# megvii-research/basedet

Hardware: AMD Instinct MI355X
Metric: images/sec training RetinaNet-R50-FPN 1333x800 (higher is better)
Workload: dtype bf16; 1 GPU; retinanet_r50_800x1344 train step (fwd+bwd+allreduce+SGD), DummyLoader boxes, random-init weights, inputs resident in HBM; per_gpu_batch=16, global_batch=16, parallelism=dp1

## Files before the change

### basedet_amd/_lib.py

```python
import ctypes as C
import os

import torch

_HERE = os.path.dirname(os.path.abspath(__file__))
LIB_PATH = os.environ.get("BASEDET_HIP_LIB") or os.path.join(_HERE, "lib", "libbasedet_hip.so")

BD_MAX_SEGS = 8
ABI_VERSION = 118
EPI_RELU, EPI_ADD_BEFORE, EPI_ADD_AFTER, EPI_MASK, EPI_SPARSE = 1, 2, 4, 8, 16


class BasedetHipError(RuntimeError):
    pass


class ConvDesc(C.Structure):
    _fields_ = [
        ("N", C.c_int32), ("Cin", C.c_int32), ("Cout", C.c_int32), ("R", C.c_int32), ("S", C.c_int32),
        ("stride", C.c_int32), ("pad", C.c_int32), ("nseg", C.c_int32),
        ("Hi", C.c_int32 * BD_MAX_SEGS), ("Wi", C.c_int32 * BD_MAX_SEGS),
        ("Ho", C.c_int32 * BD_MAX_SEGS), ("Wo", C.c_int32 * BD_MAX_SEGS),
        ("in_off", C.c_int32 * BD_MAX_SEGS), ("out_off", C.c_int32 * BD_MAX_SEGS),
        ("in_pix_per_img", C.c_int32), ("out_pix_per_img", C.c_int32),
        ("route", C.c_int32 * 4), ("sr_seed", C.c_uint32),
        ("gskip", C.c_int32), ("gskip_ws", C.c_void_p), ("gskip_ws_bytes", C.c_size_t),
        ("gskip_gmap", C.c_void_p), ("gskip_gmap_bytes", C.c_size_t), ("gskip_dxmap", C.c_void_p), ("gskip_dxmap_bytes", C.c_size_t),
        ("gskip_dx_clean", C.c_int32),
        ("fwd_map", C.c_void_p), ("fwd_map_bytes", C.c_size_t), ("fwd_clean", C.c_int32),
    ]


class PackDesc(C.Structure):
    _fields_ = [("w", C.c_void_p), ("row_scale", C.c_void_p), ("w_fwd", C.c_void_p), ("w_dgrad", C.c_void_p),
                ("Cout", C.c_int32), ("RS", C.c_int32), ("Cin", C.c_int32), ("block_start", C.c_int32)]


class ImageDesc(C.Structure):
    _fields_ = [("offset", C.c_int64), ("src_h", C.c_int32), ("src_w", C.c_int32), ("dst_h", C.c_int32), ("dst_w", C.c_int32),
                ("flip", C.c_int32), ("reserved_", C.c_int32 * 1)]


AFFINE_BRIGHTNESS, AFFINE_CONTRAST, AFFINE_SATURATION, AFFINE_LIGHTING = 1, 2, 4, 8

# ... 7 lines not shown
_P, _I, _L, _F, _Z = C.c_void_p, C.c_int, C.c_int64, C.c_float, C.c_size_t
_D = C.POINTER(ConvDesc)

SIGNATURES = {
    "bd_last_error_string": (C.c_char_p, []),
    "bd_version": (_I, []),
    "bd_conv_last_kernel": (C.c_char_p, []),
    "bd_probe_mfma_rate": (_I, [C.c_double, C.POINTER(C.c_double), C.POINTER(C.c_double), _P]),
    "bd_probe_kernel_clock": (_I, [C.c_char_p, _I, C.POINTER(C.c_double), C.POINTER(C.c_double)]),
    "bd_conv2d_fwd": (_I, [_D, _P, _P, _P, _P, _P, _I, _P]),
    "bd_conv2d_dgrad": (_I, [_D, _P, _P, _P, _P, _P, _I, _P]),
    "bd_conv2d_dgrad_gskip_bytes": (_Z, [_D]),
    "bd_conv2d_gskip_map_bytes": (_Z, [_D, _I]),
    "bd_gskip_map_scan": (_I, [_D, _I, _P, _P, _Z, _P]),
    "bd_fwd_live_map_bytes": (_Z, [_D]),
    "bd_fwd_live_maps": (_I, [_D, _P, _I, _I, C.POINTER(C.c_void_p), _Z, _I, _P]),
    "bd_conv2d_fwd_bits": (_I, [_D, _P, _P, _P, _P, _P, _P, _I, _P]),
    "bd_conv2d_fwd_ex": (_I, [_D, _P, _P, _P, _P, _P, _P, _P, _F, _I, _P]),
    "bd_conv2d_dgrad_ex": (_I, [_D, _P, _P, _P, _P, _P, _P, _P, _F, _I, _P]),
    "bd_conv2d_dgrad_bits": (_I, [_D, _P, _P, _P, _P, _P, _I, _P]),
    "bd_conv2d_wgrad_workspace_bytes": (_Z, [_D]),
    "bd_conv2d_wgrad": (_I, [_D, _P, _P, _P, _P, _I, _P, _Z, _P]),
    "bd_conv2d_wgrad_bias_workspace_bytes": (_Z, [_D]),
    "bd_conv2d_wgrad_bias": (_I, [_D, _P, _P, _P, _P, _P, _I, _P, _Z, _P]),
    "bd_fpn_deconv_pack": (_I, [_P, _I, _P, _P, _P]),
    "bd_fpn_deconv_fwd": (_I, [_P, _P, _P, _P, _I, _I, _I, _I, _I, _I, _P]),
    "bd_fpn_deconv_dgrad": (_I, [_P, _P, _P, _P, _I, _I, _I, _I, _I, _I, _P]),
    "bd_fpn_deconv_wgrad_workspace_bytes": (_Z, [_I, _I, _I, _I]),
    "bd_fpn_deconv_wgrad": (_I, [_P, _P, _P, _I, _P, _Z, _I, _I, _I, _I, _I, _I, _P]),
    "bd_deform_conv_fwd": (_I, [_P, _P, _P, _P, _P] + [_I] * 12 + [_P]),
    "bd_deform_conv_wgrad_workspace_bytes": (_Z, [_I] * 5),
# ... 222 lines not shown
```

### basedet_amd/csrc/conv3x3_pp128.hip

```cpp
#include "conv3x3_pp128_body.h"

namespace {
using namespace pp128;

struct PSeg { int patch_start, H, W, pw, src_off, dst_off; };

struct PParams {
    const bf16_raw* src;
    const bf16_raw* w;
    const float* bias;
    const bf16_raw* add;
    const bf16_raw* mask;
    bf16_raw* dst;
    int CK, CO, flags, nseg;
    int src_ppi, dst_ppi;
    unsigned src_bytes;
    int patches_per_img, total_patches, n_tiles;
    int patch_begin;
    PSeg seg[MAX_SEG];
};


template <int MODE, int TCO>
__global__ __launch_bounds__(512, 1) void conv3x3_pp128_kernel(const PParams p) {
    extern __shared__ __attribute__((aligned(16))) unsigned char smem[];
    pp128::body<MODE, TCO>(p, smem, (int)blockIdx.x, (int)gridDim.x, p.patch_begin, p.total_patches, p.n_tiles);
}

}

extern BD_KNOB int g_patch_pp128;
int bd_conv3x3_pp128_launch_range(const bd_conv_desc* d, int mode, const void* src, const void* w, const float* bias, const void* add,
                                  const void* mask, void* dst, int flags, hipStream_t stream, int patch_begin, int patch_end, int tco) {
    PParams p{};
    p.CK = mode == 0 ? d->Cin : d->Cout;
    p.CO = mode == 0 ? d->Cout : d->Cin;
    p.src_ppi = mode == 0 ? d->in_pix_per_img : d->out_pix_per_img;
    p.dst_ppi = mode == 0 ? d->out_pix_per_img : d->in_pix_per_img;
    if (p.CK % 8 != 0 || p.CO % 8 != 0) return 1;
    if ((long long)d->N * p.src_ppi * p.CK * 2 >= 0x7fffffffll || (long long)d->N * p.dst_ppi >= 0x7fffffffll ||
        (long long)p.CO * 9 * p.CK >= 0x7fffffffll) return 1;
    p.src = (const bf16_raw*)src; p.w = (const bf16_raw*)w; p.bias = bias;
    p.add = (const bf16_raw*)add; p.mask = (const bf16_raw*)mask; p.dst = (bf16_raw*)dst;
    p.flags = flags; p.nseg = d->nseg;
    p.src_bytes = (unsigned)((long long)d->N * p.src_ppi * p.CK * 2);
    int ps = 0;
    for (int s = 0; s < d->nseg; ++s) {
        PSeg& sg = p.seg[s];
        sg.patch_start = ps; sg.H = d->Ho[s]; sg.W = d->Wo[s]; sg.pw = cdiv(d->Wo[s], PW);
        sg.src_off = mode == 0 ? d->in_off[s] : d->out_off[s];
        sg.dst_off = mode == 0 ? d->out_off[s] : d->in_off[s];
        ps += cdiv(d->Ho[s], PH) * sg.pw;
    }
    p.patches_per_img = ps;
    p.total_patches = patch_end >= 0 ? patch_end : ps * d->N;
    p.patch_begin = patch_begin;
    const bool small = tco ? tco == 64 : p.CO <= 64;
    if (!tco && (g_patch_pp128 < 0 || (g_patch_pp128 == 0 && !small))) return 1;
    p.n_tiles = cdiv(p.CO, small ? 64 : 128);
    const int grid = cdiv(p.total_patches - p.patch_begin, NPATCH) * p.n_tiles;
    if (grid <= 0) return 0;
    BD_ONCE_PER_DEVICE(
        (void)hipFuncSetAttribute(reinterpret_cast<const void*>(&conv3x3_pp128_kernel<0, 128>), hipFuncAttributeMaxDynamicSharedMemorySize, Tile<128>::LDS_BYTES);
        (void)hipFuncSetAttribute(reinterpret_cast<const void*>(&conv3x3_pp128_kernel<1, 128>), hipFuncAttributeMaxDynamicSharedMemorySize, Tile<128>::LDS_BYTES);
        (void)hipFuncSetAttribute(reinterpret_cast<const void*>(&conv3x3_pp128_kernel<0, 64>), hipFuncAttributeMaxDynamicSharedMemorySize, Tile<64>::LDS_BYTES);
        (void)hipFuncSetAttribute(reinterpret_cast<const void*>(&conv3x3_pp128_kernel<1, 64>), hipFuncAttributeMaxDynamicSharedMemorySize, Tile<64>::LDS_BYTES));
    if (!tco) bd_note_kernel("conv3x3_pp128_kernel");
    if (small) {
        if (mode == 0) hipLaunchKernelGGL((conv3x3_pp128_kernel<0, 64>), dim3(grid), dim3(512), Tile<64>::LDS_BYTES, stream, p);
        else hipLaunchKernelGGL((conv3x3_pp128_kernel<1, 64>), dim3(grid), dim3(512), Tile<64>::LDS_BYTES, stream, p);
    } else {
        if (mode == 0) hipLaunchKernelGGL((conv3x3_pp128_kernel<0, 128>), dim3(grid), dim3(512), Tile<128>::LDS_BYTES, stream, p);
        else hipLaunchKernelGGL((conv3x3_pp128_kernel<1, 128>), dim3(grid), dim3(512), Tile<128>::LDS_BYTES, stream, p);
    }
    return 0;
}

int bd_conv3x3_pp128_launch(const bd_conv_desc* d, int mode, const void* src, const void* w, const float* bias, const void* add,
                            const void* mask, void* dst, int flags, hipStream_t stream) {
    return bd_conv3x3_pp128_launch_range(d, mode, src, w, bias, add, mask, dst, flags, stream, 0, -1, 0);
}
```

### basedet_amd/csrc/conv3x3_pp128_body.h

```cpp
#pragma once
#include "common.h"

namespace pp128 {


constexpr int PH = 4, PW = 16, IH = PH + 2, IW = PW + 2;
constexpr int NPATCH = 4;
constexpr int XROWS = NPATCH * IH * IW;
constexpr int X_PITCH = 144;
constexpr int X_BYTES = XROWS * X_PITCH;
constexpr int XPASSES = 7;
constexpr int NSLOT = 4;
template <int TCO> struct Tile {
    static constexpr int W_SLOT = TCO * 128;
    static constexpr int W_BYTES = NSLOT * W_SLOT;
    static constexpr int LDS_BYTES = W_BYTES + X_BYTES + TCO * 4;
    static constexpr int MREP = TCO / 32;
    static constexpr int NPIECE = TCO / 64;
};
constexpr int MAX_SEG = BD_MAX_SEGS;

typedef __attribute__((address_space(3))) void lds_void_t;
typedef __attribute__((address_space(1))) const void glb_void_t;

__device__ __forceinline__ int swz(int row, int chunk) { return row * 128 + ((chunk ^ (row & 7)) << 4); }
__device__ __forceinline__ int colperm(int f) { return f < 4 ? 2 * f : (f < 12 ? 2 * (f - 4) + 1 : 2 * (f - 8)); }
__device__ __forceinline__ int xpos(int chunk) { return (chunk >> 2) * 64 + ((((chunk & 1) << 1) | ((chunk >> 1) & 1)) << 4); }

#define PP_FENCE() __builtin_amdgcn_sched_barrier(0)
#define PP_BARRIER() do { asm volatile("" ::: "memory"); __builtin_amdgcn_s_barrier(); asm volatile("" ::: "memory"); } while (0)


template <int MODE, int TCO, class P>
__device__ __forceinline__ void body(const P& p, unsigned char* smem, int bid, const int nwg, const int patch_begin, const int patch_end, const int n_tiles) {
    constexpr int TILE_CO = TCO, W_SLOT = Tile<TCO>::W_SLOT, W_BYTES = Tile<TCO>::W_BYTES, MREP = Tile<TCO>::MREP, NPIECE = Tile<TCO>::NPIECE;
    constexpr int HALF = TCO / 2;
    unsigned char* wbuf = smem;
    unsigned char* xbuf = smem + W_BYTES;
    float* sbias = reinterpret_cast<float*>(smem + W_BYTES + X_BYTES);

    const int tid = threadIdx.x, lane = tid & 63, wave = __builtin_amdgcn_readfirstlane(tid >> 6);
    const int wm = wave >> 2, wp = wave & 3;
    {
        const int q = nwg >> 3, r = nwg & 7, xcd = bid & 7;
        bid = (xcd < r ? xcd * (q + 1) : r * (q + 1) + (xcd - r) * q) + (bid >> 3);
    }
    const int pt = bid / n_tiles;
    const int ct = bid - pt * n_tiles;
    const int co0 = ct * TILE_CO;

    int py0[NPATCH], px0[NPATCH], pH[NPATCH], pWd[NPATCH];
    int psrc[NPATCH], pdst[NPATCH];
#pragma unroll
    for (int k = 0; k < NPATCH; ++k) {
        const int pid = patch_begin + pt * NPATCH + k;
        pH[k] = 0; pWd[k] = 0; py0[k] = 0; px0[k] = 0; psrc[k] = 0; pdst[k] = 0;
        if (pid < patch_end) {
            const int n = pid / p.patches_per_img;
            const int rem = pid - n * p.patches_per_img;
            int s = 0;
#pragma unroll
            for (int q = 1; q < MAX_SEG; ++q)
                if (q < p.nseg && rem >= p.seg[q].patch_start) s = q;
            const auto sg = p.seg[s];
            const int local = rem - sg.patch_start;
            const int by = local / sg.pw, bx = local - by * sg.pw;
            py0[k] = by * PH; px0[k] = bx * PW; pH[k] = sg.H; pWd[k] = sg.W;
            psrc[k] = n * p.src_ppi + sg.src_off;
            pdst[k] = n * p.dst_ppi + sg.dst_off;
        }
// ... 226 lines not shown
```

### basedet_amd/csrc/conv_igemm.hip

```cpp
#include "igemm_params.h"

using namespace igemm;

namespace {

template <int BK>
struct Cfg {
    static constexpr int CHUNKS = BK / 8;
    static constexpr int ROWS_PER_PASS = 256 / CHUNKS;
    static constexpr int PASSES = 128 / ROWS_PER_PASS;
    static constexpr int LDS_STRIDE = BK == 64 ? 160 : 64;
    static constexpr int TILE_BYTES = 128 * LDS_STRIDE;
    __device__ static __forceinline__ int off(int row, int chunk) {
        if constexpr (BK == 64) return row * LDS_STRIDE + chunk * 16;
        else return row * 64 + ((chunk ^ ((row >> 1) & 3)) << 4);
    }
};

template <int BK, bool PRE, bool BUF>
__global__ __launch_bounds__(256) void conv_igemm_kernel(const IgemmParams p) {
    using C = Cfg<BK>;
    extern __shared__ __attribute__((aligned(16))) unsigned char smem[];
    unsigned char* tiles = smem;
    unsigned int* s_tapmask = reinterpret_cast<unsigned int*>(smem);
// ... 373 lines not shown
}
BD_KNOB int g_use_patch3x3 = 1;
#ifdef BD_AB_SKIP
BD_KNOB int g_skip_s2_3x3 = 0;
#endif
BD_KNOB int g_bk32_for_1x1 = 1;
BD_KNOB int g_bk32_s2 = 1;

}


int bd_conv3x3_patch_launch(const bd_conv_desc* d, int mode, const void* src, const void* w, const float* bias,
                            const void* add, const void* mask, void* dst, int flags, hipStream_t stream);
bool bd_conv3x3_pp_maps_ok(const bd_conv_desc* d, int flags, const void* add, const void* dst);
bool bd_conv3x3_pp_fwd_map_ok(const bd_conv_desc* d, int flags, const void* add);

extern BD_KNOB int g_patch_dma;
extern BD_KNOB int g_patch_pp;
extern BD_KNOB int g_patch_pp128;
extern BD_KNOB int g_conv1x1_s2;
extern BD_KNOB int g_pp_tail_split;
extern BD_KNOB int g_pp_persistent;
static int bd_route_patch3x3(int enable) {
#ifdef BD_AB_SKIP
    g_skip_s2_3x3 = (enable >> 4) & 1;
#else
    if ((enable >> 4) & 1) {
        bd_set_error("bd_conv_desc.route[1]: bit 4 (skip the 3x3 / stride-2 launches: a timing A/B that leaves stale outputs) exists in "
                     "-DBD_AB_SKIP diagnostic builds only");
        return BD_EINVAL;
// ... 42 lines not shown
                         const unsigned* maskbits, void* dst, int flags, hipStream_t stream);
namespace {
bool is_dense_1x1(const bd_conv_desc* d) {
    return d->R == 1 && d->S == 1 && d->stride == 1 && d->pad == 0 && d->nseg == 1 && d->in_off[0] == 0 && d->out_off[0] == 0 &&
           d->in_pix_per_img == d->Hi[0] * d->Wi[0] && d->out_pix_per_img == d->Ho[0] * d->Wo[0];
}
}

static int conv2d_fwd_impl(const bd_conv_desc* d, const void* x, const void* w_packed, const float* bias, const void* add, void* y,
                           unsigned* ybits, void* y8, float q_scale, int flags, bd_stream_t stream) {
    if (int e = check_desc(d)) return e;
    BD_REQUIRE(x && w_packed && y, "conv2d_fwd: null pointer");
    BD_REQUIRE(d->Cin % 8 == 0, "conv2d_fwd: Cin=%d must be a multiple of 8", d->Cin);
    BD_REQUIRE(d->Cout % 8 == 0, "conv2d_fwd: Cout=%d must be a multiple of 8", d->Cout);
    BD_REQUIRE(!(flags & BD_EPI_MASK), "conv2d_fwd: BD_EPI_MASK is a dgrad-only flag");
    if (d->fwd_map || d->fwd_clean) {
        BD_REQUIRE(d->fwd_map && is_3x3s1(d) && g_use_patch3x3 && !ybits && !y8 && bd_conv3x3_pp_fwd_map_ok(d, flags, add),
                   "conv2d_fwd: fwd_map needs a 3x3 / stride 1 / pad 1 descriptor into more than 128 channels without residual operand on the "
                   "default route (fwd_clean needs fwd_map)");
        BD_REQUIRE(d->fwd_map_bytes >= bd_fwd_live_map_bytes(d), "conv2d_fwd: fwd_map %zu < required %zu bytes", (size_t)d->fwd_map_bytes,
                   bd_fwd_live_map_bytes(d));
    }
    if (is_dense_1x1(d) &&
        bd_conv1x1_dense_launch(x, w_packed, bias, add, nullptr, nullptr, y, ybits, y8, q_scale, 0, (long long)d->N * d->out_pix_per_img,
                                d->Cin, d->Cout, flags, (hipStream_t)stream) == 0) {
        BD_CHECK_LAUNCH("bd_conv2d_fwd(dense 1x1)");
        return BD_OK;
    }
    if (!ybits && !y8 && d->stride == 2 && d->R == 1 &&
        bd_conv1x1_s2_launch(d, 0, x, w_packed, bias, add, nullptr, nullptr, y, flags, (hipStream_t)stream) == 0) {
        BD_CHECK_LAUNCH("bd_conv2d_fwd(1x1 stride 2)");
// ... 175 lines not shown
```

### basedet_amd/csrc/gskip.hip

```cpp
#include "common.h"

namespace {

enum { GS_ANY = 1, GS_TOP = 2, GS_BOT = 4, GS_LEFT = 8, GS_RIGHT = 16, GS_TL = 32, GS_TR = 64, GS_BL = 128, GS_BR = 256 };

struct GsSeg { int patch_start, H, W, pw, off; };

struct GsParams {
    const bf16_raw* g;
    int* mask;
    int C, ppi, ph, pw_px, nseg, patches_per_img, total;
    GsSeg seg[BD_MAX_SEGS];
};

__device__ __forceinline__ int gs_level(const GsParams& p, int rem) {
    int s = 0;
#pragma unroll
    for (int k = 1; k < BD_MAX_SEGS; ++k)
        if (k < p.nseg && rem >= p.seg[k].patch_start) s = k;
    return s;
}

__global__ __launch_bounds__(256) void gskip_scan_kernel(const GsParams p) {
    __shared__ int sbits;
// ... 201 lines not shown
    if (!slast) return;
    __builtin_amdgcn_fence(__ATOMIC_ACQUIRE, "agent");
    const int nxt = (p.map[0] & 1) ^ 1;
    int* live = m8 + p.tot8;
    gs_compact_body<true>(cp, live, live + p.tot4 * (1 + nxt), p.map + 2 + nxt, wsum);
    if (tid == 0) { p.map[0] = nxt; p.map[1] = 0; }
}

enum { FL_HDR = 8, FL_MAX_DEPTH = 8 };

struct FlSeg { int H, W, off, s4, pw; };

struct FlParams {
    const int* labels;
    int* map[FL_MAX_DEPTH];
    int A, ppi, nseg, depths, pi4, tot4;
    FlSeg seg[BD_MAX_SEGS];
};

__global__ __launch_bounds__(1024) void fwd_live_kernel(const FlParams p) {
    extern __shared__ __attribute__((aligned(16))) unsigned char fl_bm[];
    __shared__ int slast;
    __shared__ int wsum[16];
    const int tid = threadIdx.x;
    const int n = blockIdx.x / p.nseg, s = blockIdx.x - n * p.nseg;
    const int H = p.seg[s].H, W = p.seg[s].W, HW = H * W, pwn = p.seg[s].pw;
    const int npatch = ((H + 3) >> 2) * pwn;
    unsigned char* cur = fl_bm;
    unsigned char* nxt = fl_bm + HW;
    for (int i = tid; i < HW; i += 1024) cur[i] = 0;
    __syncthreads();
    const int* lab = p.labels + ((long long)n * p.ppi + p.seg[s].off) * p.A;
    for (int i = tid; i < HW * p.A; i += 1024)
        if (lab[i] > 0) cur[i / p.A] = 1;
    __syncthreads();
    for (int k = 0; k < p.depths; ++k) {
        for (int i = tid; i < HW; i += 1024) {
            const int y = i / W, x = i - y * W;
            const int y0 = y > 0 ? y - 1 : 0, y1 = y + 1 < H ? y + 1 : H - 1, x0 = x > 0 ? x - 1 : 0, x1 = x + 1 < W ? x + 1 : W - 1;
            int v = 0;
            for (int yy = y0; yy <= y1; ++yy)
                for (int xx = x0; xx <= x1; ++xx) v |= cur[yy * W + xx];
            nxt[i] = (unsigned char)v;
        }
        __syncthreads();
        int* live = p.map[k] + FL_HDR + n * p.pi4 + p.seg[s].s4;
        for (int q = tid; q < npatch; q += 1024) {
            const int by = q / pwn, bx = q - by * pwn;
            const int ye = by * 4 + 4 < H ? by * 4 + 4 : H, xe = bx * 16 + 16 < W ? bx * 16 + 16 : W;
            int v = 0;
            for (int y = by * 4; y < ye; ++y)
                for (int x = bx * 16; x < xe; ++x) v |= nxt[y * W + x];
            live[q] = v;
        }
        unsigned char* t = cur; cur = nxt; nxt = t;
        __syncthreads();
    }
    __builtin_amdgcn_fence(__ATOMIC_RELEASE, "agent");
    __syncthreads();
    if (tid == 0) slast = atomicAdd(p.map[0] + 1, 1) == (int)gridDim.x - 1;
    __syncthreads();
    if (!slast) return;
    __builtin_amdgcn_fence(__ATOMIC_ACQUIRE, "agent");
    constexpr int KP = 8;
    const int wv = tid >> 6, ln = tid & 63;
    for (int k = 0; k < p.depths; ++k) {
        int* hdr = p.map[k];
        const int* live = hdr + FL_HDR;
        const int to = (hdr[0] & 1) ^ 1;
        int* list = hdr + FL_HDR + p.tot4 * (1 + to);
        int base = 0;
        for (int c0 = 0; c0 < p.tot4; c0 += 1024 * KP) {
            int lv[KP];
            int cnt = 0;
#pragma unroll
            for (int j = 0; j < KP; ++j) {
                const int q = c0 + tid * KP + j;
                lv[j] = q < p.tot4 ? (__hip_atomic_load(live + q, __ATOMIC_RELAXED, __HIP_MEMORY_SCOPE_AGENT) != 0) : 0;
                cnt += lv[j];
            }
            int inc = cnt;
#pragma unroll
// ... 104 lines not shown
}

void bd_fwd_map_layout(const bd_conv_desc* d, BdFwdMap* out) {
    const int p4 = gs_params(d, 4, 16, 0).total;
    out->p4 = p4; out->live = FL_HDR; out->list = FL_HDR + p4;
    out->ints = (size_t)FL_HDR + (size_t)3 * p4;
}

extern "C" size_t bd_fwd_live_map_bytes(const bd_conv_desc* d) {
    if (!d || d->nseg < 1 || d->nseg > BD_MAX_SEGS || !(d->R == 3 && d->S == 3 && d->stride == 1 && d->pad == 1)) return 0;
    BdFwdMap m;
    bd_fwd_map_layout(d, &m);
    return m.ints * sizeof(int);
}

extern "C" int bd_fwd_live_maps(const bd_conv_desc* d, const int32_t* labels, int A, int depths, void* const* maps, size_t map_bytes,
                                int reset, bd_stream_t stream) {
    BD_REQUIRE(d && labels && maps, "fwd_live_maps: null pointer");
    const size_t need = bd_fwd_live_map_bytes(d);
    BD_REQUIRE(need > 0, "fwd_live_maps: forward liveness maps belong to 3x3 / stride 1 / pad 1 descriptors");
    BD_REQUIRE(A >= 1 && depths >= 1 && depths <= FL_MAX_DEPTH, "fwd_live_maps: A=%d depths=%d (1 .. %d)", A, depths, (int)FL_MAX_DEPTH);
    BD_REQUIRE(map_bytes >= need, "fwd_live_maps: map %zu < required %zu bytes", map_bytes, need);
    const GsParams g4 = gs_params(d, 4, 16, 0);
    FlParams p{};
    p.labels = labels; p.A = A; p.ppi = g4.ppi; p.nseg = g4.nseg; p.depths = depths; p.pi4 = g4.patches_per_img; p.tot4 = g4.total;
    size_t lds = 0;
    for (int s = 0; s < g4.nseg; ++s) {
        BD_REQUIRE(d->Hi[s] == d->Ho[s] && d->Wi[s] == d->Wo[s], "fwd_live_maps: level %d changes size", s);
        p.seg[s] = FlSeg{g4.seg[s].H, g4.seg[s].W, g4.seg[s].off, g4.seg[s].patch_start, g4.seg[s].pw};
        const size_t b = (size_t)2 * g4.seg[s].H * g4.seg[s].W;
        BD_REQUIRE((long long)g4.seg[s].H * g4.seg[s].W * A < 0x7fffffffll, "fwd_live_maps: level %d too large", s);
        lds = b > lds ? b : lds;
    }
    BD_REQUIRE(lds <= 160 * 1024 - 256, "fwd_live_maps: a level of %zu pixels does not fit the LDS bitmap", lds / 2);
    for (int k = 0; k < depths; ++k) {
        BD_REQUIRE(maps[k], "fwd_live_maps: null map %d", k);
        p.map[k] = (int*)maps[k];
        if (reset && hipMemsetAsync(maps[k], 0, FL_HDR * sizeof(int), (hipStream_t)stream) != hipSuccess) {
            bd_set_error("fwd_live_maps: memset failed");
            return BD_ELAUNCH;
        }
    }
    if (d->N < 1 || g4.total < 1) return BD_OK;
    BD_ONCE_PER_DEVICE((void)hipFuncSetAttribute(reinterpret_cast<const void*>(&fwd_live_kernel), hipFuncAttributeMaxDynamicSharedMemorySize,
                                                 160 * 1024 - 256));
    hipLaunchKernelGGL(fwd_live_kernel, dim3(d->N * g4.nseg), dim3(1024), lds, (hipStream_t)stream, p);
    BD_CHECK_LAUNCH("bd_fwd_live_maps");
    return BD_OK;
}
// ... 1 lines not shown
```

### basedet_amd/models/engine.py

```python
import numpy as np
import torch

from .. import ops
from ..ops import Geom

BN_EPS = 1e-5


class ParamArena:

    def __init__(self, device):
        self.device = device
        self.entries = []
        self.total = 0
        self.w = self.g = self.v = None

    def reserve(self, name, shape):
        n = int(np.prod(shape))
        off = self.total
        self.entries.append((name, tuple(shape), off, n))
        self.total += (n + 63) // 64 * 64
        return len(self.entries) - 1

    def allocate(self):
# ... 151 lines not shown
            h = self._gskip_cache[id(d)] = (ops.gskip_desc(d, self._gskip_ws), d)
        gmap, dxmap, clean = self._chain
        if gmap is None and dxmap is None:
            return h[0]
        key = (id(d), self._gskip_ws.data_ptr(), gmap.data_ptr() if gmap is not None else 0, dxmap.data_ptr() if dxmap is not None else 0, clean)
        c = self._chain_cache.get(key)
        if c is None:
            if len(self._chain_cache) > 64:
                self._chain_cache.clear()
            c = self._chain_cache[key] = (ops.gskip_desc(d, self._gskip_ws, gmap=gmap, dxmap=dxmap, dx_clean=clean), d)
        return c[0]

    def set_chain(self, gmap=None, dxmap=None, dx_clean=False):
        self._chain = (gmap, dxmap, bool(dx_clean) and dxmap is not None) if self.gskip else (None, None, False)

    def fwd_map_desc(self, gin: Geom, gout: Geom, fmap, clean):
        d = self.desc(gin, gout)
        key = (id(d), fmap.data_ptr(), bool(clean))
        c = self._fwd_map_cache.get(key)
        if c is None:
            if len(self._fwd_map_cache) > 64:
                self._fwd_map_cache.clear()
            c = self._fwd_map_cache[key] = (ops.fwd_map_desc(d, fmap, clean), d)
        return c[0]

    def forward(self, x, gin, gout, y, add=None, relu=False, bits=None, x8=None, y8=None, q_scale=1.0, fwd_map=None, fwd_clean=False):
        flags = (ops.EPI_RELU if relu else 0) | (ops.EPI_ADD_BEFORE if add is not None else 0)
        if fwd_map is not None:
            assert not self.fp8 and not self.fp8_1x1 and bits is None and y8 is None
            return ops.conv2d_fwd(self.fwd_map_desc(gin, gout, fwd_map, fwd_clean), x, self.w_fwd, self.b, y, add=add, flags=flags)
        if self.fp8_1x1 and x8 is not None and ops.conv1x1_fp8_ok(self.desc(gin, gout), 0):
            return ops.conv1x1_fp8(self.desc(gin, gout), 0, x8, self.w_q8, self.w_scale8, self.b, y, add=add, bits=bits, y8=y8,
                                   q_scale=q_scale, flags=flags)
        if self.fp8 and bits is None:
            xq = x8 if x8 is not None else ops.quantize_fp8(x, self.act_scale, self.q8_scratch(x.numel())[: x.numel()])
            return ops.conv2d_fwd_fp8(self.desc(gin, gout), xq, self.w_q8, self.w_scale8, self.b, y, add=add, flags=flags, y8=y8,
                                      q_scale=self.act_scale)
        return ops.conv2d_fwd(self.desc(gin, gout), x, self.w_fwd, self.b, y, add=add, flags=flags, bits=bits,
                              y8=y8 if (y8 is not None and ops.dense_1x1_bits_ok(self.desc(gin, gout))) else None, q_scale=q_scale)

    def gnstats_ok(self):
        return (not self.fp8) and self.k == 3 and self.stride == 1 and self.pad == 1 and self.cout == 256 and self.cin % 64 == 0

    def forward_gnstats(self, x, gin, gout, y, part):
        return ops.conv2d_fwd_gnstats(self.desc(gin, gout), x, self.w_fwd, self.b, y, part)
# ... 249 lines not shown
```

### basedet_amd/models/retinanet.py

```python
import torch

from .. import ops
from ..streams import fork, join
from ..utils.registry import registers
from . import params as P
from .engine import PaddedClsConv
from .fpn_base import FPNDetector, _round_up


@registers.models.register()
class RetinaNet(FPNDetector):
    READS_MATCHER = True

    @staticmethod
    def init_params(cfg, seed=0):
        return P.init_retinanet_params(cfg, seed)

    @classmethod
    def check_config(cls, cfg):
        super().check_config(cfg)
        cls.check_anchor_config(cfg, matcher=cls.READS_MATCHER)
        if not cfg.MODEL.HEAD.get("WITH_NORM", True):
            raise ValueError("MODEL.HEAD.WITH_NORM = False is not supported for the RetinaNet family: only True (the default) is implemented")

# ... 3 lines not shown
        self.num_anchors = len(m.ANCHOR.SCALES[0]) * len(m.ANCHOR.RATIOS[0])
        nc = m.HEAD.NUM_CONVS
        self.cls_tower = [add(f"head.cls_subnet.{2 * i}", ch, ch, 3, 1, 1, bias=True) for i in range(nc)]
        self.box_tower = [add(f"head.bbox_subnet.{2 * i}", ch, ch, 3, 1, 1, bias=True) for i in range(nc)]
        A, K = self.num_anchors, self.num_classes
        self.cls_score = self.convs["head.cls_score"] = PaddedClsConv("head.cls_score", ch, A, K, 3, 1, 1, self.device)
        self.cls_ld = self.cls_score.cls_ld
        self.box_ld = _round_up(A * 4, 8)
        self.bbox_pred = add("head.bbox_pred", ch, A * 4, 3, 1, 1, bias=True, cout_pad=self.box_ld)
        if bool(m.get("SPARSE_BOX_BWD", True)) and m.get("WEIGHT_DTYPE", "bf16") == "bf16":
            for c in self.box_tower + [self.bbox_pred]:
                c.gskip = True
        self.sparse_chain = bool(m.get("SPARSE_BOX_CHAIN", True))
        self.sparse_box_fwd = (bool(m.get("SPARSE_BOX_FWD", True)) and type(self) is RetinaNet and nc >= 1 and nc <= 8
                               and all(c.gskip for c in self.box_tower + [self.bbox_pred]))
        self._build_base_anchors()

    def _head_convs(self):
        return self.cls_tower + self.box_tower + [self.cls_score, self.bbox_pred]

    def _plan_head(self, pl):
        ch = self.fpn_ch
        N = pl.N
        C = pl._carve
        bf = torch.bfloat16

        def act(g, c):
            return C.empty((g.pixels, c), bf)

        nc = len(self.cls_tower)
# ... 3 lines not shown
        pl.logits = act(pl.pyr, A * self.cls_ld)
        pl.offsets = act(pl.pyr, self.box_ld)
        pl.d_logits = C.like(pl.logits)
        pl.d_offsets = C.like(pl.offsets)
        pl.g_tower = [[act(pl.pyr, ch) for _ in range(nc)] for _ in range(2)]
        pl.g_map = None
        if self.sparse_chain and all(c.gskip for c in self.box_tower + [self.bbox_pred]):
            nb = ops.conv2d_gskip_map_bytes(self.box_tower[0].desc(pl.pyr, pl.pyr))
            if nb:
                pl.g_map = [C.empty(((nb + 3) // 4,), torch.int32) for _ in range(nc)]
        pl.chain_epoch = None
        pl.f_map = None
        if self.sparse_box_fwd:
            nb = ops.fwd_live_map_bytes(self.box_tower[0].desc(pl.pyr, pl.pyr))
            if nb:
                pl.f_map = [C.empty(((nb + 3) // 4,), torch.int32) for _ in range(nc)]
        pl.fwd_epoch = None
        pl.fwd_skip = None
        pl.fwd_skipped = False
        tw = lambda: C.empty((pl.pyr.pixels, ch), torch.uint8)
        pl.cls_act8 = [tw() if c.fp8 else None for c in self.cls_tower]
        pl.box_act8 = [tw() if c.fp8 else None for c in self.box_tower]
        tg = self.fp8_grad_twins
        pl.g_tower8 = [[tw() if (c.fp8_dgrad and tg) else None for c in tower] for tower in (self.cls_tower, self.box_tower)]
        pl.g_P8 = tw() if (tg and all(t[0].fp8_dgrad for t in (self.cls_tower, self.box_tower))) else None
        self._plan_anchors(pl)
        tot = pl.A_total
        pl.labels = C.empty((N, tot), torch.int32)
        pl.match_idx = C.empty((N, tot), torch.int32)
        pl.gt_offsets = C.empty((N, tot, 4), torch.float32)
        pl.num_fg = C.zeros((1,), torch.int32)
# ... 4 lines not shown
        side = self.streams.aux() if concurrent else None
        skip, pl.fwd_skip = pl.fwd_skip, None
        if skip is not None and side is None:
            join(self.streams.aux_stream)
        if skip is None:
            pl.fwd_epoch = None
        pl.fwd_skipped = skip is not None
        with fork(side):
            t, t8 = pl.P, getattr(pl, "P8", None)
            for i, (c, a, a8) in enumerate(zip(self.box_tower, pl.box_act, pl.box_act8)):
                if skip is not None:
                    c.forward(t, pl.pyr, pl.pyr, a, relu=True, fwd_map=pl.f_map[i], fwd_clean=skip[0])
                else:
                    c.forward(t, pl.pyr, pl.pyr, a, relu=True, x8=t8, y8=a8)
                t, t8 = a, a8
            self.bbox_pred.forward(t, pl.pyr, pl.pyr, pl.offsets, x8=t8)
        t, t8 = pl.P, getattr(pl, "P8", None)
        for c, a, a8 in zip(self.cls_tower, pl.cls_act, pl.cls_act8):
            c.forward(t, pl.pyr, pl.pyr, a, relu=True, x8=t8, y8=a8); t, t8 = a, a8
        self.cls_score.forward(t, pl.pyr, pl.pyr, pl.logits, x8=t8)
        join(side)

    def get_losses(self, inputs):
        assert self.training
        pre = self.pre_process(inputs)
        pl = pre["plan"]
        self._cur = pl
        m = self.cfg.MODEL
        gt = pre["gt_boxes"]
        num_gt = pre["img_info"][:, 4].to(torch.int32).contiguous()
        N, Gmax = gt.shape[0], gt.shape[1]
        ws = self._scratch("assign", N * Gmax * 4).view(torch.float32)
        thr = m.MATCHER.THRESHOLDS
        side = self.streams.aux() if m.get("ASSIGN_ON_SIDE_STREAM", True) else None
        with fork(side):
            ops.retina_assign_encode(pl.anchors, gt, num_gt, thr[0], thr[1], m.MATCHER.ALLOW_LOW_QUALITY, m.BOX_REG.MEAN,
                                     m.BOX_REG.STD, pl.labels, pl.match_idx, pl.gt_offsets, pl.num_fg, ws)
            if pl.f_map is not None and self.streams.aux() is not None:
                clean = pl.fwd_epoch == self.plan_arena.epoch
                pl.fwd_epoch = self.plan_arena.epoch
                ops.fwd_live_maps(self.box_tower[0].desc(pl.pyr, pl.pyr), pl.labels, self.num_anchors, pl.f_map[::-1], reset=not clean)
                pl.fwd_skip = (clean,)
        self.network_forward(pl)
        join(side)
        pl.loss_buf.zero_()
        rows = N * pl.A_total
        ops.focal_loss_fwd_bwd(pl.logits, pl.labels, rows, self.num_classes, m.LOSSES.FOCAL_LOSS_ALPHA,
                               m.LOSSES.FOCAL_LOSS_GAMMA, pl.num_fg, 1.0, pl.loss_buf[0:1], pl.d_logits, ld=self.cls_ld)
        ops.smooth_l1_fwd_bwd(pl.offsets, pl.gt_offsets, pl.labels, pl.pyr.pixels, self.num_anchors, self.box_ld,
                              m.LOSSES.SMOOTH_L1_BETA, pl.num_fg, m.LOSSES.REG_LOSS_WEIGHT, pl.loss_buf[1:2], pl.d_offsets)
        cls_loss, reg_loss = pl.loss_buf[0], pl.loss_buf[1]
        return {"total_loss": cls_loss + reg_loss, "cls_loss": cls_loss, "reg_loss": reg_loss}

    def head_backward(self, pl, ws, cws):
        pyr = pl.pyr
        for ti, (tower, acts, pred, dpred) in enumerate(((self.cls_tower, pl.cls_act, self.cls_score, pl.d_logits),
# ... 59 lines not shown
```

### basedet_amd/ops.py

```python
import ctypes as C
from dataclasses import dataclass, field
from typing import List, Optional

import torch

from . import _lib
from ._lib import ConvDesc, EPI_ADD_AFTER, EPI_ADD_BEFORE, EPI_MASK, EPI_RELU, EPI_SPARSE, check, f32arr, i32arr, ptr, stream_ptr


@dataclass
class Geom:
    N: int
    H: List[int]
    W: List[int]
    off: List[int] = field(default_factory=list)
    pix_per_img: int = 0

    def __post_init__(self):
        if not self.off:
            o = 0
            self.off = []
            for h, w in zip(self.H, self.W):
                self.off.append(o)
                o += h * w
# ... 107 lines not shown
        h.gskip_ws_bytes = scratch.numel() * scratch.element_size()
    if gmap is not None:
        h.gskip_gmap = gmap.data_ptr()
        h.gskip_gmap_bytes = gmap.numel() * gmap.element_size()
    if dxmap is not None:
        h.gskip_dxmap = dxmap.data_ptr()
        h.gskip_dxmap_bytes = dxmap.numel() * dxmap.element_size()
    h.gskip_dx_clean = int(bool(dx_clean))
    return h


def fwd_live_map_bytes(d):
    return int(L().bd_fwd_live_map_bytes(C.byref(d)))


def fwd_live_maps(d, labels, A, maps, reset=False):
    if labels.dtype != torch.int32 or labels.numel() != d.N * d.out_pix_per_img * A:
        raise _lib.BasedetHipError(f"fwd_live_maps: labels must be int32 with N * pixels * A = {d.N * d.out_pix_per_img * A} entries")
    nb = min(m.numel() * m.element_size() for m in maps)
    arr = (C.c_void_p * len(maps))(*[ptr(m).value for m in maps])
    check(L().bd_fwd_live_maps(C.byref(d), ptr(labels), int(A), len(maps), arr, nb, int(bool(reset)), stream_ptr()), "bd_fwd_live_maps")
    return maps


def fwd_map_desc(d, fmap, clean=False):
    h = ConvDesc.from_buffer_copy(d)
    h.fwd_map = fmap.data_ptr()
    h.fwd_map_bytes = fmap.numel() * fmap.element_size()
    h.fwd_clean = int(bool(clean))
    return h


def quantize_fp8(x, scale, q):
    check(L().bd_quantize_fp8(ptr(x), x.numel(), float(scale), ptr(q), stream_ptr()), "bd_quantize_fp8")
    return q


def weight_pack_fp8(w, row_scale, Cout, RS, Cin, act_scale, wq, wscale):
    check(L().bd_weight_pack_fp8(ptr(w), ptr(row_scale), Cout, RS, Cin, float(act_scale), ptr(wq), ptr(wscale), stream_ptr()),
          "bd_weight_pack_fp8")


def conv2d_fwd_fp8(d, xq, wq, wscale, bias, y, add=None, flags=0, y8=None, q_scale=1.0):
    check(L().bd_conv2d_fwd_fp8_ex(C.byref(_stamp(d)), ptr(xq), ptr(wq), ptr(wscale), ptr(bias), ptr(add), ptr(y), ptr(y8), float(q_scale), flags,
# ... 985 lines not shown
```

### include/basedet_hip.h

```cpp
#ifndef BASEDET_HIP_H
#define BASEDET_HIP_H

#include <stddef.h>
#include <stdint.h>

#ifdef __cplusplus
extern "C" {
#endif

#define BD_OK 0
#define BD_EINVAL (-1)
#define BD_ELAUNCH (-2)
#define BD_EWORKSPACE (-3)

#define BD_MAX_SEGS 8

#define BD_EPI_RELU 1
#define BD_EPI_ADD_BEFORE 2
#define BD_EPI_ADD_AFTER 4
#define BD_EPI_MASK 8
#define BD_EPI_SPARSE 16

typedef void* bd_stream_t;

// ... 8 lines not shown
    int32_t in_off[BD_MAX_SEGS], out_off[BD_MAX_SEGS];
    int32_t in_pix_per_img, out_pix_per_img;
    int32_t route[4];
    uint32_t sr_seed;
    int32_t gskip;
    void* gskip_ws;
    size_t gskip_ws_bytes;
    void* gskip_gmap;
    size_t gskip_gmap_bytes;
    void* gskip_dxmap;
    size_t gskip_dxmap_bytes;
    int32_t gskip_dx_clean;
    void* fwd_map;
    size_t fwd_map_bytes;
    int32_t fwd_clean;
} bd_conv_desc;

const char* bd_last_error_string(void);
int bd_version(void);
const char* bd_conv_last_kernel(void);
int bd_probe_mfma_rate(double seconds, double* tflops_out, double* clock_mhz_out, bd_stream_t stream);

int bd_probe_kernel_clock(const char* kernel, int reset, double* clock_mhz_out, double* busy_ms_out);


int bd_conv2d_fwd(const bd_conv_desc* d, const void* x, const void* w_packed, const float* bias,
                  const void* add, void* y, int flags, bd_stream_t stream);

int bd_conv2d_dgrad(const bd_conv_desc* d, const void* g, const void* w_packed_t, const void* add,
                    const void* mask, void* dx, int flags, bd_stream_t stream);
size_t bd_conv2d_dgrad_gskip_bytes(const bd_conv_desc* d);
size_t bd_conv2d_gskip_map_bytes(const bd_conv_desc* d, int of_dx);
int bd_gskip_map_scan(const bd_conv_desc* d, int of_dx, const void* t, void* map, size_t map_bytes, bd_stream_t stream);
size_t bd_fwd_live_map_bytes(const bd_conv_desc* d);
int bd_fwd_live_maps(const bd_conv_desc* d, const int32_t* labels, int A, int depths, void* const* maps, size_t map_bytes, int reset,
                     bd_stream_t stream);

int bd_conv2d_fwd_bits(const bd_conv_desc* d, const void* x, const void* w_packed, const float* bias, const void* add, void* y,
                       uint32_t* ybits, int flags, bd_stream_t stream);
int bd_conv2d_dgrad_bits(const bd_conv_desc* d, const void* g, const void* w_packed_t, const void* add, const uint32_t* maskbits,
                         void* dx, int flags, bd_stream_t stream);
int bd_conv2d_fwd_ex(const bd_conv_desc* d, const void* x, const void* w_packed, const float* bias, const void* add, void* y,
                     uint32_t* ybits, void* y8, float q_scale, int flags, bd_stream_t stream);
int bd_conv2d_dgrad_ex(const bd_conv_desc* d, const void* g, const void* w_packed_t, const void* add, const void* mask,
                       const uint32_t* maskbits, void* dx, void* dx8, float q_scale, int flags, bd_stream_t stream);

size_t bd_conv2d_wgrad_workspace_bytes(const bd_conv_desc* d);
int bd_conv2d_wgrad(const bd_conv_desc* d, const void* x, const void* g, const float* row_scale, float* dw,
                    int accumulate, void* ws, size_t ws_bytes, bd_stream_t stream);

size_t bd_conv2d_wgrad_bias_workspace_bytes(const bd_conv_desc* d);
// ... 466 lines not shown
```

Measured before the change: 724.7 images/sec.

## Compute box-regression prediction conv only on patches with positive anchors

Adds a sparse forward path for the bbox_pred 3x3 conv (at most 64 output channels). A new depth-0 liveness map marks 4x16 patches that contain anchors with positive labels, and the kernel runs the pp128 body only over the listed live patches. It zero-fills dead patches, and when clean it only re-zeros patches that were live on the previous step. The goal is to skip dense conv work on regions whose box outputs never reach the loss, in exchange for an extra map build and list indirection in the kernel. If any consumer reads box predictions at non-positive anchors, the output is no longer the same as the dense result.

```diff
diff --git a/basedet_amd/_lib.py b/basedet_amd/_lib.py
--- a/basedet_amd/_lib.py
+++ b/basedet_amd/_lib.py
@@ -28,6 +28,7 @@
         ("gskip_gmap", C.c_void_p), ("gskip_gmap_bytes", C.c_size_t), ("gskip_dxmap", C.c_void_p), ("gskip_dxmap_bytes", C.c_size_t),
         ("gskip_dx_clean", C.c_int32),
         ("fwd_map", C.c_void_p), ("fwd_map_bytes", C.c_size_t), ("fwd_clean", C.c_int32),
+        ("fwd_pred", C.c_int32),
     ]
 
 
@@ -65,7 +66,7 @@
     "bd_conv2d_gskip_map_bytes": (_Z, [_D, _I]),
     "bd_gskip_map_scan": (_I, [_D, _I, _P, _P, _Z, _P]),
     "bd_fwd_live_map_bytes": (_Z, [_D]),
-    "bd_fwd_live_maps": (_I, [_D, _P, _I, _I, C.POINTER(C.c_void_p), _Z, _I, _P]),
+    "bd_fwd_live_maps": (_I, [_D, _P, _I, _I, C.POINTER(C.c_void_p), _P, _Z, _I, _P]),
     "bd_conv2d_fwd_bits": (_I, [_D, _P, _P, _P, _P, _P, _P, _I, _P]),
     "bd_conv2d_fwd_ex": (_I, [_D, _P, _P, _P, _P, _P, _P, _P, _F, _I, _P]),
     "bd_conv2d_dgrad_ex": (_I, [_D, _P, _P, _P, _P, _P, _P, _P, _F, _I, _P]),
diff --git a/basedet_amd/csrc/conv3x3_pp128.hip b/basedet_amd/csrc/conv3x3_pp128.hip
--- a/basedet_amd/csrc/conv3x3_pp128.hip
+++ b/basedet_amd/csrc/conv3x3_pp128.hip
@@ -25,6 +25,56 @@
 __global__ __launch_bounds__(512, 1) void conv3x3_pp128_kernel(const PParams p) {
     extern __shared__ __attribute__((aligned(16))) unsigned char smem[];
     pp128::body<MODE, TCO>(p, smem, (int)blockIdx.x, (int)gridDim.x, p.patch_begin, p.total_patches, p.n_tiles);
+}
+
+struct SpFwd {
+    const int* hdr;
+    const int* live;
+    const int* list;
+    int stride, clean;
+};
+
+__global__ __launch_bounds__(512, 1) void conv3x3_pp128_fwd_sparse_kernel(const PParams p, const SpFwd s) {
+    extern __shared__ __attribute__((aligned(16))) unsigned char smem[];
+    const int cur = __builtin_amdgcn_readfirstlane(s.hdr[0] & 1);
+    int count = __builtin_amdgcn_readfirstlane(s.hdr[2 + cur]);
+    count = count < 0 ? 0 : (count > p.total_patches ? p.total_patches : count);
+    const int tiles = (count + NPATCH - 1) / NPATCH;
+    const int grid = (int)gridDim.x, bid = (int)blockIdx.x;
+    if (bid < tiles) pp128::body<0, 64, true>(p, smem, bid, tiles, 0, p.total_patches, 1, s.list + (long long)cur * s.stride, count);
+    int z, nz;
+    if (tiles < grid) {
+        if (bid < tiles) return;
+        z = bid - tiles; nz = grid - tiles;
+    } else {
+        z = bid; nz = grid;
+    }
+    int nprev = __builtin_amdgcn_readfirstlane(s.hdr[2 + (cur ^ 1)]);
+    nprev = nprev < 0 ? 0 : (nprev > p.total_patches ? p.total_patches : nprev);
+    const int* prev = s.list + (long long)(cur ^ 1) * s.stride;
+    const int n = s.clean ? nprev : p.total_patches;
+    const int tid = threadIdx.x;
+    const int cpp = p.CO >> 3;
+    for (int i = z; i < n; i += nz) {
+        const int q = s.clean ? prev[i] : i;
+        if ((unsigned)q >= (unsigned)p.total_patches || s.live[q] != 0) continue;
+        const int im = q / p.patches_per_img, rem = q - im * p.patches_per_img;
+        int sgi = 0;
+#pragma unroll
+        for (int k = 1; k < MAX_SEG; ++k)
+            if (k < p.nseg && rem >= p.seg[k].patch_start) sgi = k;
+        const PSeg sg = p.seg[sgi];
+        const int local = rem - sg.patch_start, by = local / sg.pw, bx = local - by * sg.pw;
+        const int y0 = by * PH, x0 = bx * PW;
+        const int wpx = x0 + PW <= sg.W ? PW : sg.W - x0;
+        const int rowc = wpx * cpp;
+        for (int c = tid; c < PH * rowc; c += 512) {
+            const int r = c / rowc, cc = c - r * rowc;
+            if (y0 + r >= sg.H) break;
+            const long long pix = (long long)im * p.dst_ppi + sg.dst_off + (long long)(y0 + r) * sg.W + x0;
+            *reinterpret_cast<u32x4_t*>(p.dst + pix * p.CO + cc * 8) = (u32x4_t){0u, 0u, 0u, 0u};
+        }
+    }
 }
 
 }
@@ -55,7 +105,19 @@
     p.patches_per_img = ps;
     p.total_patches = patch_end >= 0 ? patch_end : ps * d->N;
     p.patch_begin = patch_begin;
-    const bool small = tco ? tco == 64 : p.CO <= 64;
+    if (mode == 0 && d->fwd_map && d->fwd_pred && !tco) {
+        BdFwdMap fm;
+        bd_fwd_map_layout(d, &fm);
+        const int* m = (const int*)d->fwd_map;
+        const SpFwd s{m, m + fm.live, m + fm.list, p.total_patches, d->fwd_clean ? 1 : 0};
+        p.n_tiles = 1;
+        BD_ONCE_PER_DEVICE((void)hipFuncSetAttribute(reinterpret_cast<const void*>(&conv3x3_pp128_fwd_sparse_kernel),
+                                                     hipFuncAttributeMaxDynamicSharedMemorySize, Tile<64>::LDS_BYTES));
+        bd_note_kernel("conv3x3_pp128_kernel");
+        hipLaunchKernelGGL(conv3x3_pp128_fwd_sparse_kernel, dim3(cdiv(p.total_patches, NPATCH)), dim3(512), Tile<64>::LDS_BYTES, stream, p, s);
+        return 0;
+    }
+    const bool small =tco ? tco == 64 : p.CO <= 64;
     if (!tco && (g_patch_pp128 < 0 || (g_patch_pp128 == 0 && !small))) return 1;
     p.n_tiles = cdiv(p.CO, small ? 64 : 128);
     const int grid = cdiv(p.total_patches - p.patch_begin, NPATCH) * p.n_tiles;
@@ -76,6 +138,20 @@
     return 0;
 }
 
+bool bd_conv3x3_pp128_fwd_map_ok(const bd_conv_desc* d, int flags, const void* add) {
+    if (g_patch_pp128 < 0 || !(d->R == 3 && d->S == 3 && d->stride == 1 && d->pad == 1)) return false;
+    if (d->Cin % 8 != 0 || d->Cout > 64 || d->Cout % 8 != 0) return false;
+    if ((long long)d->N * d->in_pix_per_img * d->Cin * 2 >= 0x7fffffffll || (long long)d->N * d->out_pix_per_img >= 0x7fffffffll ||
+        (long long)d->Cin * 9 * d->Cout >= 0x7fffffffll) return false;
+    long long patches = 0;
+    for (int s = 0; s < d->nseg; ++s) {
+        if (d->Hi[s] != d->Ho[s] || d->Wi[s] != d->Wo[s]) return false;
+        patches += (long long)cdiv(d->Ho[s], PH) * cdiv(d->Wo[s], PW);
+    }
+    if (patches < 1 || patches * d->N >= (1 << 24)) return false;
+    return !add && !(flags & ~BD_EPI_RELU);
+}
+
 int bd_conv3x3_pp128_launch(const bd_conv_desc* d, int mode, const void* src, const void* w, const float* bias, const void* add,
                             const void* mask, void* dst, int flags, hipStream_t stream) {
     return bd_conv3x3_pp128_launch_range(d, mode, src, w, bias, add, mask, dst, flags, stream, 0, -1, 0);
diff --git a/basedet_amd/csrc/conv3x3_pp128_body.h b/basedet_amd/csrc/conv3x3_pp128_body.h
--- a/basedet_amd/csrc/conv3x3_pp128_body.h
+++ b/basedet_amd/csrc/conv3x3_pp128_body.h
@@ -31,8 +31,9 @@
 #define PP_BARRIER() do { asm volatile("" ::: "memory"); __builtin_amdgcn_s_barrier(); asm volatile("" ::: "memory"); } while (0)
 
 
-template <int MODE, int TCO, class P>
-__device__ __forceinline__ void body(const P& p, unsigned char* smem, int bid, const int nwg, const int patch_begin, const int patch_end, const int n_tiles) {
+template <int MODE, int TCO, bool LIST = false, class P>
+__device__ __forceinline__ void body(const P& p, unsigned char* smem, int bid, const int nwg, const int patch_begin, const int patch_end, const int n_tiles,
+                                     const int* plist = nullptr, const int plist_n = 0) {
     constexpr int TILE_CO = TCO, W_SLOT = Tile<TCO>::W_SLOT, W_BYTES = Tile<TCO>::W_BYTES, MREP = Tile<TCO>::MREP, NPIECE = Tile<TCO>::NPIECE;
     constexpr int HALF = TCO / 2;
     unsigned char* wbuf = smem;
@@ -53,7 +54,8 @@
     int psrc[NPATCH], pdst[NPATCH];
 #pragma unroll
     for (int k = 0; k < NPATCH; ++k) {
-        const int pid = patch_begin + pt * NPATCH + k;
+        int pid = patch_begin + pt * NPATCH + k;
+        if constexpr (LIST) pid = pid < plist_n ? plist[pid] : patch_end;
         pH[k] = 0; pWd[k] = 0; py0[k] = 0; px0[k] = 0; psrc[k] = 0; pdst[k] = 0;
         if (pid < patch_end) {
             const int n = pid / p.patches_per_img;
diff --git a/basedet_amd/csrc/conv_igemm.hip b/basedet_amd/csrc/conv_igemm.hip
--- a/basedet_amd/csrc/conv_igemm.hip
+++ b/basedet_amd/csrc/conv_igemm.hip
@@ -411,6 +411,7 @@
                             const void* add, const void* mask, void* dst, int flags, hipStream_t stream);
 bool bd_conv3x3_pp_maps_ok(const bd_conv_desc* d, int flags, const void* add, const void* dst);
 bool bd_conv3x3_pp_fwd_map_ok(const bd_conv_desc* d, int flags, const void* add);
+bool bd_conv3x3_pp128_fwd_map_ok(const bd_conv_desc* d, int flags, const void* add);
 
 extern BD_KNOB int g_patch_dma;
 extern BD_KNOB int g_patch_pp;
@@ -483,7 +484,13 @@
     BD_REQUIRE(d->Cin % 8 == 0, "conv2d_fwd: Cin=%d must be a multiple of 8", d->Cin);
     BD_REQUIRE(d->Cout % 8 == 0, "conv2d_fwd: Cout=%d must be a multiple of 8", d->Cout);
     BD_REQUIRE(!(flags & BD_EPI_MASK), "conv2d_fwd: BD_EPI_MASK is a dgrad-only flag");
-    if (d->fwd_map || d->fwd_clean) {
+    if (d->fwd_pred) {
+        BD_REQUIRE(d->fwd_map && is_3x3s1(d) && g_use_patch3x3 && !ybits && !y8 && bd_conv3x3_pp128_fwd_map_ok(d, flags, add),
+                   "conv2d_fwd: fwd_pred needs fwd_map on a 3x3 / stride 1 / pad 1 descriptor into at most 64 channels without residual operand "
+                   "on the default route");
+        BD_REQUIRE(d->fwd_map_bytes >= bd_fwd_live_map_bytes(d), "conv2d_fwd: fwd_map %zu < required %zu bytes", (size_t)d->fwd_map_bytes,
+                   bd_fwd_live_map_bytes(d));
+    } else if (d->fwd_map || d->fwd_clean) {
         BD_REQUIRE(d->fwd_map && is_3x3s1(d) && g_use_patch3x3 && !ybits && !y8 && bd_conv3x3_pp_fwd_map_ok(d, flags, add),
                    "conv2d_fwd: fwd_map needs a 3x3 / stride 1 / pad 1 descriptor into more than 128 channels without residual operand on the "
                    "default route (fwd_clean needs fwd_map)");
diff --git a/basedet_amd/csrc/gskip.hip b/basedet_amd/csrc/gskip.hip
--- a/basedet_amd/csrc/gskip.hip
+++ b/basedet_amd/csrc/gskip.hip
@@ -239,6 +239,7 @@
 struct FlParams {
     const int* labels;
     int* map[FL_MAX_DEPTH];
+    int* map0;
     int A, ppi, nseg, depths, pi4, tot4;
     FlSeg seg[BD_MAX_SEGS];
 };
@@ -259,6 +260,17 @@
     for (int i = tid; i < HW * p.A; i += 1024)
         if (lab[i] > 0) cur[i / p.A] = 1;
     __syncthreads();
+    if (p.map0) {
+        int* live = p.map0 + FL_HDR + n * p.pi4 + p.seg[s].s4;
+        for (int q = tid; q < npatch; q += 1024) {
+            const int by = q / pwn, bx = q - by * pwn;
+            const int ye = by * 4 + 4 < H ? by * 4 + 4 : H, xe = bx * 16 + 16 < W ? bx * 16 + 16 : W;
+            int v = 0;
+            for (int y = by * 4; y < ye; ++y)
+                for (int x = bx * 16; x < xe; ++x) v |= cur[y * W + x];
+            live[q] = v;
+        }
+    }
     for (int k = 0; k < p.depths; ++k) {
         for (int i = tid; i < HW; i += 1024) {
             const int y = i / W, x = i - y * W;
@@ -289,8 +301,8 @@
     __builtin_amdgcn_fence(__ATOMIC_ACQUIRE, "agent");
     constexpr int KP = 8;
     const int wv = tid >> 6, ln = tid & 63;
-    for (int k = 0; k < p.depths; ++k) {
-        int* hdr = p.map[k];
+    for (int k = p.map0 ? -1 : 0; k < p.depths; ++k) {
+        int* hdr = k < 0 ? p.map0 : p.map[k];
         const int* live = hdr + FL_HDR;
         const int to = (hdr[0] & 1) ^ 1;
         int* list = hdr + FL_HDR + p.tot4 * (1 + to);
@@ -425,8 +437,8 @@
     return m.ints * sizeof(int);
 }
 
-extern "C" int bd_fwd_live_maps(const bd_conv_desc* d, const int32_t* labels, int A, int depths, void* const* maps, size_t map_bytes,
-                                int reset, bd_stream_t stream) {
+extern "C" int bd_fwd_live_maps(const bd_conv_desc* d, const int32_t* labels, int A, int depths, void* const* maps, void* map0,
+                                size_t map_bytes, int reset, bd_stream_t stream) {
     BD_REQUIRE(d && labels && maps, "fwd_live_maps: null pointer");
     const size_t need = bd_fwd_live_map_bytes(d);
     BD_REQUIRE(need > 0, "fwd_live_maps: forward liveness maps belong to 3x3 / stride 1 / pad 1 descriptors");
@@ -434,7 +446,7 @@
     BD_REQUIRE(map_bytes >= need, "fwd_live_maps: map %zu < required %zu bytes", map_bytes, need);
     const GsParams g4 = gs_params(d, 4, 16, 0);
     FlParams p{};
-    p.labels = labels; p.A = A; p.ppi = g4.ppi; p.nseg = g4.nseg; p.depths = depths; p.pi4 = g4.patches_per_img; p.tot4 = g4.total;
+    p.labels = labels; p.map0 = (int*)map0; p.A = A; p.ppi = g4.ppi; p.nseg = g4.nseg; p.depths = depths; p.pi4 = g4.patches_per_img; p.tot4 = g4.total;
     size_t lds = 0;
     for (int s = 0; s < g4.nseg; ++s) {
         BD_REQUIRE(d->Hi[s] == d->Ho[s] && d->Wi[s] == d->Wo[s], "fwd_live_maps: level %d changes size", s);
@@ -444,6 +456,10 @@
         lds = b > lds ? b : lds;
     }
     BD_REQUIRE(lds <= 160 * 1024 - 256, "fwd_live_maps: a level of %zu pixels does not fit the LDS bitmap", lds / 2);
+    if (map0 && reset && hipMemsetAsync(map0, 0, FL_HDR * sizeof(int), (hipStream_t)stream) != hipSuccess) {
+        bd_set_error("fwd_live_maps: memset failed");
+        return BD_ELAUNCH;
+    }
     for (int k = 0; k < depths; ++k) {
         BD_REQUIRE(maps[k], "fwd_live_maps: null map %d", k);
         p.map[k] = (int*)maps[k];
diff --git a/basedet_amd/models/engine.py b/basedet_amd/models/engine.py
--- a/basedet_amd/models/engine.py
+++ b/basedet_amd/models/engine.py
@@ -189,21 +189,21 @@
     def set_chain(self, gmap=None, dxmap=None, dx_clean=False):
         self._chain = (gmap, dxmap, bool(dx_clean) and dxmap is not None) if self.gskip else (None, None, False)
 
-    def fwd_map_desc(self, gin: Geom, gout: Geom, fmap, clean):
+    def fwd_map_desc(self, gin: Geom, gout: Geom, fmap, clean, pred=False):
         d = self.desc(gin, gout)
-        key = (id(d), fmap.data_ptr(), bool(clean))
+        key = (id(d), fmap.data_ptr(), bool(clean), bool(pred))
         c = self._fwd_map_cache.get(key)
         if c is None:
             if len(self._fwd_map_cache) > 64:
                 self._fwd_map_cache.clear()
-            c = self._fwd_map_cache[key] = (ops.fwd_map_desc(d, fmap, clean), d)
+            c = self._fwd_map_cache[key] = (ops.fwd_map_desc(d, fmap, clean, pred), d)
         return c[0]
 
-    def forward(self, x, gin, gout, y, add=None, relu=False, bits=None, x8=None, y8=None, q_scale=1.0, fwd_map=None, fwd_clean=False):
+    def forward(self, x, gin, gout, y, add=None, relu=False, bits=None, x8=None, y8=None, q_scale=1.0, fwd_map=None, fwd_clean=False, fwd_pred=False):
         flags = (ops.EPI_RELU if relu else 0) | (ops.EPI_ADD_BEFORE if add is not None else 0)
         if fwd_map is not None:
             assert not self.fp8 and not self.fp8_1x1 and bits is None and y8 is None
-            return ops.conv2d_fwd(self.fwd_map_desc(gin, gout, fwd_map, fwd_clean), x, self.w_fwd, self.b, y, add=add, flags=flags)
+            return ops.conv2d_fwd(self.fwd_map_desc(gin, gout, fwd_map, fwd_clean, fwd_pred), x, self.w_fwd, self.b, y, add=add, flags=flags)
         if self.fp8_1x1 and x8 is not None and ops.conv1x1_fp8_ok(self.desc(gin, gout), 0):
             return ops.conv1x1_fp8(self.desc(gin, gout), 0, x8, self.w_q8, self.w_scale8, self.b, y, add=add, bits=bits, y8=y8,
                                    q_scale=q_scale, flags=flags)
diff --git a/basedet_amd/models/retinanet.py b/basedet_amd/models/retinanet.py
--- a/basedet_amd/models/retinanet.py
+++ b/basedet_amd/models/retinanet.py
@@ -41,6 +41,7 @@
         self.sparse_chain = bool(m.get("SPARSE_BOX_CHAIN", True))
         self.sparse_box_fwd = (bool(m.get("SPARSE_BOX_FWD", True)) and type(self) is RetinaNet and nc >= 1 and nc <= 8
                                and all(c.gskip for c in self.box_tower + [self.bbox_pred]))
+        self.sparse_box_pred = self.sparse_box_fwd and bool(m.get("SPARSE_BOX_PRED", True)) and self.box_ld <= 64
         self._build_base_anchors()
 
     def _head_convs(self):
@@ -74,7 +75,7 @@
         if self.sparse_box_fwd:
             nb = ops.fwd_live_map_bytes(self.box_tower[0].desc(pl.pyr, pl.pyr))
             if nb:
-                pl.f_map = [C.empty(((nb + 3) // 4,), torch.int32) for _ in range(nc)]
+                pl.f_map = [C.empty(((nb + 3) // 4,), torch.int32) for _ in range(nc + (1 if self.sparse_box_pred else 0))]
         pl.fwd_epoch = None
         pl.fwd_skip = None
         pl.fwd_skipped = False
@@ -109,7 +110,10 @@
                 else:
                     c.forward(t, pl.pyr, pl.pyr, a, relu=True, x8=t8, y8=a8)
                 t, t8 = a, a8
-            self.bbox_pred.forward(t, pl.pyr, pl.pyr, pl.offsets, x8=t8)
+            if skip is not None and self.sparse_box_pred:
+                self.bbox_pred.forward(t, pl.pyr, pl.pyr, pl.offsets, fwd_map=pl.f_map[len(self.box_tower)], fwd_clean=skip[0], fwd_pred=True)
+            else:
+                self.bbox_pred.forward(t, pl.pyr, pl.pyr, pl.offsets, x8=t8)
         t, t8 = pl.P, getattr(pl, "P8", None)
         for c, a, a8 in zip(self.cls_tower, pl.cls_act, pl.cls_act8):
             c.forward(t, pl.pyr, pl.pyr, a, relu=True, x8=t8, y8=a8); t, t8 = a, a8
@@ -134,7 +138,9 @@
             if pl.f_map is not None and self.streams.aux() is not None:
                 clean = pl.fwd_epoch == self.plan_arena.epoch
                 pl.fwd_epoch = self.plan_arena.epoch
-                ops.fwd_live_maps(self.box_tower[0].desc(pl.pyr, pl.pyr), pl.labels, self.num_anchors, pl.f_map[::-1], reset=not clean)
+                nc = len(self.box_tower)
+                ops.fwd_live_maps(self.box_tower[0].desc(pl.pyr, pl.pyr), pl.labels, self.num_anchors, pl.f_map[nc - 1::-1], reset=not clean,
+                                  map0=pl.f_map[nc] if self.sparse_box_pred else None)
                 pl.fwd_skip = (clean,)
         self.network_forward(pl)
         join(side)
diff --git a/basedet_amd/ops.py b/basedet_amd/ops.py
--- a/basedet_amd/ops.py
+++ b/basedet_amd/ops.py
@@ -145,20 +145,22 @@
     return int(L().bd_fwd_live_map_bytes(C.byref(d)))
 
 
-def fwd_live_maps(d, labels, A, maps, reset=False):
+def fwd_live_maps(d, labels, A, maps, reset=False, map0=None):
     if labels.dtype != torch.int32 or labels.numel() != d.N * d.out_pix_per_img * A:
         raise _lib.BasedetHipError(f"fwd_live_maps: labels must be int32 with N * pixels * A = {d.N * d.out_pix_per_img * A} entries")
-    nb = min(m.numel() * m.element_size() for m in maps)
+    nb = min(m.numel() * m.element_size() for m in list(maps) + ([map0] if map0 is not None else []))
     arr = (C.c_void_p * len(maps))(*[ptr(m).value for m in maps])
-    check(L().bd_fwd_live_maps(C.byref(d), ptr(labels), int(A), len(maps), arr, nb, int(bool(reset)), stream_ptr()), "bd_fwd_live_maps")
+    check(L().bd_fwd_live_maps(C.byref(d), ptr(labels), int(A), len(maps), arr, ptr(map0), nb, int(bool(reset)), stream_ptr()),
+          "bd_fwd_live_maps")
     return maps
 
 
-def fwd_map_desc(d, fmap, clean=False):
+def fwd_map_desc(d, fmap, clean=False, pred=False):
     h = ConvDesc.from_buffer_copy(d)
     h.fwd_map = fmap.data_ptr()
     h.fwd_map_bytes = fmap.numel() * fmap.element_size()
     h.fwd_clean = int(bool(clean))
+    h.fwd_pred = int(bool(pred))
     return h
 
 
diff --git a/include/basedet_hip.h b/include/basedet_hip.h
--- a/include/basedet_hip.h
+++ b/include/basedet_hip.h
@@ -46,6 +46,7 @@
     void* fwd_map;
     size_t fwd_map_bytes;
     int32_t fwd_clean;
+    int32_t fwd_pred;
 } bd_conv_desc;
 
 const char* bd_last_error_string(void);
@@ -65,8 +66,8 @@
 size_t bd_conv2d_gskip_map_bytes(const bd_conv_desc* d, int of_dx);
 int bd_gskip_map_scan(const bd_conv_desc* d, int of_dx, const void* t, void* map, size_t map_bytes, bd_stream_t stream);
 size_t bd_fwd_live_map_bytes(const bd_conv_desc* d);
-int bd_fwd_live_maps(const bd_conv_desc* d, const int32_t* labels, int A, int depths, void* const* maps, size_t map_bytes, int reset,
-                     bd_stream_t stream);
+int bd_fwd_live_maps(const bd_conv_desc* d, const int32_t* labels, int A, int depths, void* const* maps, void* map0, size_t map_bytes,
+                     int reset, bd_stream_t stream);
 
 int bd_conv2d_fwd_bits(const bd_conv_desc* d, const void* x, const void* w_packed, const float* bias, const void* add, void* y,
                        uint32_t* ybits, int flags, bd_stream_t stream);
```

Measured after the change: 727.3 images/sec, median of 6. No clear change (+0.4%).
